# ami-iit/paper_gorbani_2025_humanoids_multi-rate-mpc-ironcub

Measured on AMD Instinct MI355X. Metric: MPC solves/sec (whole node) + p50 single-solve latency, iRonCub paper horizon, higher is better.
Workload: dtype f64

## Files before the change

### paper_gorbani_2025_humanoids_multi-rate-mpc-ironcub_amd/build.py

```python
from __future__ import annotations

import os
import shutil
import subprocess

HERE = os.path.dirname(os.path.abspath(__file__))
CSRC = os.path.join(HERE, "csrc")
LIB_PATH = os.path.join(HERE, "libvsmpc.so")
SOLVE = "vsmpc_kernels.hip"
SOURCES = [SOLVE, "vsmpc_dispatch.hip", "vsmpc_rollout.hip", "vsmpc_capi.hip", "vsmpc_jet.hip", "vsmpc_provider.hip",
           "vsmpc_runtime.hip"]
HEADERS = ["vsmpc_device.hpp", "vsmpc_launch.hpp", "vsmpc_p0.hpp", "vsmpc_smem.hpp", "vsmpc_p1_syrk.hpp", "vsmpc_p1_struct.hpp",
           "vsmpc_p3.hpp", "vsmpc_p4.hpp", "vsmpc_p5.hpp", "vsmpc_panel_asm.inc",
           "vsmpc_runtime_body.inc", "vsmpc_jet_device.hpp", "vsmpc_horizons.def", os.path.join("..", "..", "include", "vsmpc.h"),
           os.path.join("..", "..", "include", "vsmpc_jet.h")]


DEFAULT_HORIZONS = ((17, 7, 12), (34, 14, 24), (21, 9, 15))
HORIZONS_DEF = os.path.join(CSRC, "vsmpc_horizons.def")


def horizons():
    env = os.environ.get("VSMPC_HORIZONS", "").strip()
    if not env:
# ... 25 lines not shown


OBJ_DIR = os.path.join(HERE, "build")


SCHED_MAX_ILP = ["-mllvm", "-amdgpu-sched-strategy=max-ilp"]


def _units():
    units = []
    for n, ns, hc in horizons():
        sched = SCHED_MAX_ILP if n <= 24 else []
        for st in (0, 1):
            units.append((f"kernels_{n}_{ns}_{hc}_{'diag' if st else 'prod'}", SOLVE,
                          [f"-DVS_TU_HORIZON={n},{ns},{hc}", f"-DVS_TU_STAMPS={st}"] + sched))
    for src in SOURCES:
        if src != SOLVE:
            units.append((os.path.splitext(src)[0], src, []))
    return units


def _deps(src):
    return [os.path.join(CSRC, src)] + [os.path.join(CSRC, h) for h in HEADERS] + [os.path.abspath(__file__)]


def _extra_flags():
    return os.environ.get("VSMPC_HIPCC_FLAGS", "").split()


def needs_build() -> bool:
# ... 80 lines not shown
```

### paper_gorbani_2025_humanoids_multi-rate-mpc-ironcub_amd/csrc/vsmpc_capi.hip

```cpp
#include <algorithm>
#include <cmath>
#include <cstddef>
#include <cstdio>
#include <cstdlib>
#include <cstring>
#include <new>
#include <vector>

#include "vsmpc_launch.hpp"
#include "../../include/vsmpc_jet.h"

using namespace vsmpc;

struct vsmpc_handle {
    vsmpc_config cfg;
    DevCfg dev;
    int variant;
    int runtime;
    RtDims rt;
    double* d_ws;
    int sens;
    RtDims rts;
    double* d_sws;
    double* d_sdx;
    double* d_sdfm;
    int* d_sact;
    int* d_sflags;
    int form;
    KinOpts kin;
    int device;
    int max_batch;
    int n_var, n_con, n_in, n_p;
    double* d_in;
    double* d_x;
    double* d_fm;
    int* d_status;
    int* d_iters;
    double* d_lin;
    double* d_dbg;
    double* d_kin;
    double* d_kout;
    unsigned long long* d_stamps;
    hipEvent_t ev0, ev1;
// ... 57 lines not shown
}

#define HIP_TRY(expr)                                   \
    do {                                                \
        hipError_t _e = (expr);                         \
        if (_e != hipSuccess) return hip_fail(_e, #expr); \
    } while (0)

#define ON_DEVICE(dev) DeviceScope _scope(dev); HIP_TRY(_scope.err)

hipError_t solve_launch(const vsmpc_handle* h, const double* d_in, int batch, double* d_x, double* d_fm, int* d_status,
                        int* d_iters, size_t first, hipStream_t s) {
    if (h->runtime)
        return launch_solve_runtime(h->rt, h->dev, d_in, batch, h->d_ws + first * size_t(h->rt.ws_doubles), d_x, d_fm,
                                    d_status, d_iters, s);
    return launch_solve(h->variant, h->form, h->dev, d_in, batch, d_x, d_fm, d_status, d_iters, nullptr, nullptr, nullptr, s);
}

struct Stage {
    double* in; double* x; double* fm; int* st; int* it; double* kin;
};
Stage stage_view(const vsmpc_handle* h, double* base) {
    Stage v;
    v.in = base;
    v.x = v.in + size_t(ZC_MAX) * h->n_in;
    v.fm = v.x + size_t(ZC_MAX) * h->n_var;
    v.st = reinterpret_cast<int*>(v.fm + size_t(ZC_MAX) * VSMPC_FM_SIZE);
    v.it = v.st + ZC_MAX;
    v.kin = v.fm + size_t(ZC_MAX) * (VSMPC_FM_SIZE + 1);
    return v;
// ... 181 lines not shown
        if (h->pipe_done[i]) (void)hipEventDestroy(h->pipe_done[i]);
    }
    if (h->pipe_start) (void)hipEventDestroy(h->pipe_start);
    if (h->h_stage) (void)hipHostFree(h->h_stage);
    if (h->ev0) (void)hipEventDestroy(h->ev0);
    if (h->ev1) (void)hipEventDestroy(h->ev1);
    delete h;
}

int vsmpc_num_variables(const vsmpc_handle* h) { return h ? h->n_var : VSMPC_ERR_INVALID_ARG; }
int vsmpc_num_constraints(const vsmpc_handle* h) { return h ? h->n_con : VSMPC_ERR_INVALID_ARG; }
int vsmpc_input_doubles(const vsmpc_handle* h) { return h ? h->n_in : VSMPC_ERR_INVALID_ARG; }
int vsmpc_max_batch(const vsmpc_handle* h) { return h ? h->max_batch : VSMPC_ERR_INVALID_ARG; }
int vsmpc_condensed_dim(const vsmpc_handle* h) { return h ? h->n_p : VSMPC_ERR_INVALID_ARG; }
const char* vsmpc_kernel_name(const vsmpc_handle* h) {
    return h ? (h->runtime ? runtime_kernel_name() : variant_kernel_name(h->variant)) : "none";
}

int vsmpc_solve_batch_device(vsmpc_handle* h, const double* d_in, int batch, double* d_x, double* d_first_move,
                             int* d_status, int* d_iters, void* stream) {
    if (h == nullptr || d_in == nullptr || d_status == nullptr || batch < 0) return VSMPC_ERR_INVALID_ARG;
    if (batch > h->max_batch) return VSMPC_ERR_BATCH_TOO_LARGE;
    if (batch == 0) return VSMPC_OK;
    ON_DEVICE(h->device);
    HIP_TRY(solve_launch(h, d_in, batch, d_x, d_first_move, d_status, d_iters, 0, static_cast<hipStream_t>(stream)));
    return VSMPC_OK;
}

int vsmpc_solve_batch(vsmpc_handle* h, const double* in, int batch, double* x, double* first_move, int* status,
                      int* iters, void* stream) {
    if (h == nullptr || in == nullptr || status == nullptr || batch < 0) return VSMPC_ERR_INVALID_ARG;
// ... 216 lines not shown
            } else {
                lo[r1 + i * NTH + r] = h->dev.vmin;
                hi[r1 + i * NTH + r] = h->dev.vmax;
            }
        }
    return VSMPC_OK;
}

int vsmpc_debug_condensed(vsmpc_handle* h, const double* in_one, double* M, double* Lfac) {
    if (h == nullptr || in_one == nullptr) return VSMPC_ERR_INVALID_ARG;
    if (h->runtime) return VSMPC_ERR_UNSUPPORTED_CONFIG;
    ON_DEVICE(h->device);
    const size_t np2 = size_t(h->n_p) * h->n_p;
    HIP_TRY(hipMemcpy(h->d_in, in_one, h->n_in * sizeof(double), hipMemcpyHostToDevice));
    HIP_TRY(hipMemset(h->d_dbg, 0, 2 * np2 * sizeof(double)));
    HIP_TRY(launch_solve(h->variant, h->form, h->dev, h->d_in, 1, h->d_x, h->d_fm, h->d_status, h->d_iters, h->d_dbg,
                         h->d_dbg + np2, nullptr, nullptr));
    HIP_TRY(hipDeviceSynchronize());
    if (M) HIP_TRY(hipMemcpy(M, h->d_dbg, np2 * sizeof(double), hipMemcpyDeviceToHost));
    if (Lfac) HIP_TRY(hipMemcpy(Lfac, h->d_dbg + np2, np2 * sizeof(double), hipMemcpyDeviceToHost));
    return VSMPC_OK;
}

int vsmpc_kinematics_batch(vsmpc_handle* h, const double* kin, int batch, double* out, double* records) {
    if (h == nullptr || kin == nullptr || out == nullptr || batch < 0) return VSMPC_ERR_INVALID_ARG;
    if (batch > h->max_batch) return VSMPC_ERR_BATCH_TOO_LARGE;
    if (batch == 0) return VSMPC_OK;
    ON_DEVICE(h->device);
    HIP_TRY(hipMemcpy(h->d_kin, kin, size_t(batch) * VSMPC_KIN_SIZE * sizeof(double), hipMemcpyHostToDevice));
    HIP_TRY(launch_kinematics(h->d_kin, batch, h->d_kout, h->kin, nullptr));
// ... 85 lines not shown
            if (joint_selector[i] < 0 || joint_selector[i] >= VSMPC_KIN_NJ) return VSMPC_ERR_INVALID_ARG;
        for (int i = 0; i < VSMPC_N_JOINTS; ++i) h->kin.sel[i] = joint_selector[i];
    }
    h->kin.constant_lambda = constant_lambda ? 1 : 0;
    return VSMPC_OK;
}

int vsmpc_debug_phase_cycles(vsmpc_handle* h, const double* in, int batch, unsigned long long* stamps16) {
    if (h == nullptr || in == nullptr || stamps16 == nullptr || batch <= 0) return VSMPC_ERR_INVALID_ARG;
    if (h->runtime) return VSMPC_ERR_UNSUPPORTED_CONFIG;
    if (batch > h->max_batch) return VSMPC_ERR_BATCH_TOO_LARGE;
    ON_DEVICE(h->device);
    unsigned long long* d_st = h->d_stamps;
    HIP_TRY(hipMemset(d_st, 0, size_t(batch) * 16 * sizeof(unsigned long long)));
    HIP_TRY(hipMemcpy(h->d_in, in, size_t(batch) * h->n_in * sizeof(double), hipMemcpyHostToDevice));
    for (int rep = 0; rep < 3; ++rep)
        HIP_TRY(launch_solve(h->variant, h->form, h->dev, h->d_in, batch, h->d_x, h->d_fm, h->d_status, h->d_iters, nullptr,
                             nullptr, d_st, nullptr));
    HIP_TRY(hipDeviceSynchronize());
    HIP_TRY(hipMemcpy(stamps16, d_st, size_t(batch) * 16 * sizeof(unsigned long long), hipMemcpyDeviceToHost));
    return VSMPC_OK;
}

int vsmpc_timing_begin(vsmpc_handle* h, void* stream) {
    if (h == nullptr) return VSMPC_ERR_INVALID_ARG;
    HIP_TRY(hipEventRecord(h->ev0, static_cast<hipStream_t>(stream)));
    return VSMPC_OK;
}

int vsmpc_timing_end(vsmpc_handle* h, void* stream, int launches, float* ms_per_launch) {
// ... 250 lines not shown
int vsmpc_rollout_get_state(vsmpc_rollout* r, double* state) {
    if (r == nullptr || state == nullptr) return VSMPC_ERR_INVALID_ARG;
    ON_DEVICE(r->h->device);
    HIP_TRY(hipMemcpy(state, r->d_state, size_t(r->batch) * VSMPC_PLANT_STATE * sizeof(double), hipMemcpyDeviceToHost));
    return VSMPC_OK;
}

int vsmpc_rollout_get_records(vsmpc_rollout* r, double* records) {
    if (r == nullptr || records == nullptr) return VSMPC_ERR_INVALID_ARG;
    ON_DEVICE(r->h->device);
    HIP_TRY(hipMemcpy(records, r->d_rec, size_t(r->batch) * r->h->n_in * sizeof(double), hipMemcpyDeviceToHost));
    return VSMPC_OK;
}

int vsmpc_set_kernel_form(vsmpc_handle* h, int form) {
    if (h == nullptr || form < 0 || form > 2) return VSMPC_ERR_INVALID_ARG;
    if (h->runtime && form != 0) return VSMPC_ERR_UNSUPPORTED_CONFIG;
    if (form == 1 && !variant_has_structured(h->variant)) return VSMPC_ERR_UNSUPPORTED_CONFIG;
    const int prev = h->form;
    h->form = form;
    return prev;
}

void* vsmpc_alloc_host(size_t bytes) {
    void* p = nullptr;
    if (bytes == 0 || hipHostMalloc(&p, bytes, hipHostMallocDefault) != hipSuccess) { (void)hipGetLastError(); return nullptr; }
    return p;
}

void vsmpc_free_host(void* p) {
    if (p != nullptr) (void)hipHostFree(p);
}

// ... 14 lines not shown
```

### paper_gorbani_2025_humanoids_multi-rate-mpc-ironcub_amd/csrc/vsmpc_dispatch.hip

```cpp
#include <cstdlib>

#include "vsmpc_launch.hpp"
#include "vsmpc_smem.hpp"

namespace vsmpc {

__global__ __launch_bounds__(64) void kinematics_kernel(const double* __restrict__ kin, int batch,
                                                        double* __restrict__ out, KinOpts opts) {
    __shared__ __attribute__((aligned(16))) double s[VSMPC_KIN_SIZE + 1];
    __shared__ double sRa[12], sRr[12];
    const int b = blockIdx.x, lane = threadIdx.x;
    if (b >= batch) return;
    const double* rec = kin + size_t(b) * VSMPC_KIN_SIZE;
    const int head = (reinterpret_cast<size_t>(rec) & 15) ? 1 : 0;
    if (lane == 0 && head) s[0] = rec[0];
    const double2* r2 = reinterpret_cast<const double2*>(rec + head);
    const int n2 = (VSMPC_KIN_SIZE - head) / 2;
    for (int i = lane; i < n2; i += 64) {
        const double2 v = r2[i];
        s[head + 2 * i] = v.x;
        s[head + 2 * i + 1] = v.y;
    }
    if (lane == 0 && ((VSMPC_KIN_SIZE - head) & 1)) s[VSMPC_KIN_SIZE - 1] = rec[VSMPC_KIN_SIZE - 1];
    __syncthreads();
// ... 65 lines not shown
hipError_t launch_kinematics(const double* d_kin, int batch, double* d_out, const KinOpts& opts, hipStream_t stream) {
    hipLaunchKernelGGL(kinematics_kernel, dim3(batch), dim3(64), 0, stream, d_kin, batch, d_out, opts);
    return hipGetLastError();
}

int initial_kernel_form() {
    const char* v = getenv("VSMPC_FORM");
    return (v != nullptr && v[0] == 's' && v[1] == 't') ? 1 : (v != nullptr && v[0] == 's' && v[1] == 'y') ? 2 : 0;
}

struct HorizonEntry {
    int n_iter, n_iter_small, control_horizon, n_p;
    size_t lds_bytes;
    const char* name;
    bool structured;
};
#define VSMPC_STR2(x) #x
#define VSMPC_STR(x) VSMPC_STR2(x)
static const HorizonEntry kHorizons[] = {
#define X(N, NS, HC) {N, NS, HC, Dims<N, NS, HC>::NP, Dims<N, NS, HC>::STRUCT_P1 ? Smem<Dims<N, NS, HC>>::bytes_struct : Smem<Dims<N, NS, HC>>::bytes, "solve_kernel<Dims<" VSMPC_STR(N) "," VSMPC_STR(NS) "," VSMPC_STR(HC) ">>", Dims<N, NS, HC>::STRUCT_P1},
#include "vsmpc_horizons.def"
#undef X
};
constexpr int kNumHorizons = int(sizeof(kHorizons) / sizeof(kHorizons[0]));

int select_variant(int n_iter, int n_iter_small, int control_horizon) {
    for (int i = 0; i < kNumHorizons; ++i)
        if (kHorizons[i].n_iter == n_iter && kHorizons[i].n_iter_small == n_iter_small &&
            kHorizons[i].control_horizon == control_horizon)
            return i + 1;
    return VARIANT_NONE;
}

int num_variants() { return kNumHorizons; }

void variant_horizon(int variant, int* n_iter, int* n_iter_small, int* control_horizon) {
    const HorizonEntry& h = kHorizons[variant - 1];
    *n_iter = h.n_iter;
    *n_iter_small = h.n_iter_small;
    *control_horizon = h.control_horizon;
}

const char* variant_kernel_name(int variant) {
    return (variant >= 1 && variant <= kNumHorizons) ? kHorizons[variant - 1].name : "none";
}

int variant_condensed_dim(int variant) {
    return (variant >= 1 && variant <= kNumHorizons) ? kHorizons[variant - 1].n_p : 0;
}

bool variant_has_structured(int variant) {
    return variant >= 1 && variant <= kNumHorizons && kHorizons[variant - 1].structured;
}

size_t variant_lds_bytes(int variant) {
    return (variant >= 1 && variant <= kNumHorizons) ? kHorizons[variant - 1].lds_bytes : 0;
}

hipError_t launch_solve(int variant, int form, const DevCfg& cfg, const double* d_in, int batch, double* d_x, double* d_fm,
                        int* d_status, int* d_iters, double* dbgM, double* dbgL, unsigned long long* stamps,
                        hipStream_t stream) {
    int id = 0;
#define X(N, NS, HC)                                                                                                  \
// ... 24 lines not shown
```

### paper_gorbani_2025_humanoids_multi-rate-mpc-ironcub_amd/csrc/vsmpc_kernels.hip

```cpp
#include <atomic>

#include "vsmpc_launch.hpp"
#include "vsmpc_p0.hpp"
#include "vsmpc_p1_syrk.hpp"
#include "vsmpc_p1_struct.hpp"
#include "vsmpc_p3.hpp"
#include "vsmpc_p4.hpp"
#include "vsmpc_p5.hpp"

#if !defined(VS_TU_HORIZON) || !defined(VS_TU_STAMPS)
#error "one unit per horizon: -DVS_TU_HORIZON=N,NS,HC -DVS_TU_STAMPS=0|1 (build.py)"
#endif

namespace vsmpc {

template <class D, int K0 = 0, int K1 = NJC>
VS_DEV void p0_joint_reduction(double* __restrict__ sm, int lane) {
    using S = Smem<D>;
    static_assert(VSMPC_IN_LANG == VSMPC_IN_LLIN + 24, "Lambda_lin and Lambda_ang are adjacent in the record");
    const double* sIn = sm + S::oIn;
    const double* sCfg = sm + S::oCfg;
    double* sBj = sm + S::oBj;
    double* sQR = sm + S::oQR;
    const int c = lane < 6 ? lane : 6;
    double a[8];
    if constexpr (K0 == 0) {
// ... 117 lines not shown
    double* xout;
    double* fmout;
    int* status_out;
    int* iters_out;
    double* dbgM;
    double* dbgL;
    unsigned long long* stamps;
};
VS_DEV const SolveArgs* late_args() {
    const SolveArgs* ka = reinterpret_cast<const SolveArgs*>(
        (const void*)__builtin_amdgcn_kernarg_segment_ptr());
    asm volatile("" : "+s"(ka));
    return ka;
}

template <class D, bool STAMPS, int FORM = 0>
__global__ __launch_bounds__(D::BLOCK, D::WG_PER_CU) void solve_kernel(DevCfg cfg, const double* __restrict__ in, int batch,
                                                         double* xout_, double* fmout_, int* status_out_,
                                                         int* iters_out_, double* dbgM_, double* dbgL_,
                                                         unsigned long long* stamps_) {
#define VS_STAMP(i)                                                                         \
    do {                                                                                    \
        if constexpr (STAMPS) {                                                             \
            unsigned long long* st_ = late_args()->stamps;                                  \
            if (tid == 0 && st_ != nullptr) st_[size_t(blockIdx.x) * 16 + (i)] = __builtin_amdgcn_s_memtime(); \
        }                                                                                   \
    } while (0)
    unsigned long long t_acc[6] = {0, 0, 0, 0, 0, 0};
    unsigned long long t_mark = 0, stamp_t1 = 0, rt0 = 0;
    if constexpr (STAMPS) rt0 = __builtin_amdgcn_s_memrealtime();
#define VS_TIC()                                                     \
    do {                                                             \
        if constexpr (STAMPS) t_mark = __builtin_amdgcn_s_memtime(); \
    } while (0)
#define VS_TOC(i)                                                          \
    do {                                                                   \
        if constexpr (STAMPS) {                                            \
            const unsigned long long t_now = __builtin_amdgcn_s_memtime(); \
            t_acc[i] += t_now - t_mark;                                    \
            t_mark = t_now;                                                \
        }                                                                  \
    } while (0)
    using S = Smem<D>;
    constexpr bool FUSED_DISPATCH = FORM == 1;
    constexpr bool PIPE = FORM == 1;
    constexpr int QR_P0_STEPS = D::STRUCT_LONG ? 1 : 2;
    extern __shared__ __attribute__((aligned(16))) double smem[];
    double* sIn = smem + S::oIn;
    double* sA = smem + S::oA;
    double* sBj = smem + S::oBj;
    double* sBt = smem + S::oBt;
    double* sC = smem + S::oC;
    double* sVprev = smem + S::oVprev;
    double* sInvD = smem + S::oInvD;
    double* sW = smem + S::oW;
    double* sZ = smem + S::oZ;
    double* sSv = smem + S::oSv;
    double* sSvec = smem + S::oSvec;
    double* sV = smem + S::oV;
    double* sX = smem + S::oX;
// ... 32 lines not shown
        if (tid < D::NIN / 2) rec = in2[tid];
        if (tid < 4) sFlags[tid] = 0;
        if (tid < D::N) sDt[tid] = cfg.dt[tid];
        if (tid >= 64 && tid < 64 + NWROWS) sCfg[CFG_SQ + tid - 64] = cfg.sq[tid - 64];
        if (tid >= 96 && tid < 96 + NJ) sCfg[CFG_WJ + tid - 96] = cfg.wj[tid - 96];
        if (tid == 128) {
            sCfg[CFG_WREG] = cfg.w_reg; sCfg[CFG_WTHR] = cfg.w_thr; sCfg[CFG_WINIT] = cfg.w_init;
            sCfg[CFG_VMIN] = cfg.vmin; sCfg[CFG_VMAX] = cfg.vmax;
        }
        for (int i = tid; i < NX * NX + NX * NJ + NX * NTH + 28; i += D::BLOCK) sA[i] = 0.0;
        if (tid < D::NIN / 2) sIn2[tid] = rec;
    }
    __syncthreads();
    p0_linearize<D, false, false, false>(cfg.use_jet, sIn, sA, sBj, sBt, sC, sVprev, tid, D::BLOCK);
    if (wave == 3) {
        if constexpr (FORM == 1) p0_joint_reduction<D, 0, QR_P0_STEPS>(smem, lane);
        else p0_joint_reduction<D>(smem, lane);
    }

    constexpr int NJROW = D::NV + NTH + 1, ZROW = D::NV + NTH;
    double* sJetT = sXinv;
    double* sGA = sJetT + NJROW * D::N;
    static_assert(D::NV + NTH <= 64 && NJROW * D::N + 6 * D::N <= S::NXT * D::TS, "jet trajectories fit the X region");
    if (wave == 1) {
        if (lane < D::NV + NTH) {
            const bool affl = lane >= D::NV;
            const int i = affl ? lane - D::NV : (lane & 3);
            const int blk = affl ? -1 : v_block_of_internal<D>(lane);
            const double jon = sA[(12 + i) * NX + 16 + i], ja = sA[(16 + i) * NX + 12 + i], jb = sA[(16 + i) * NX + 16 + i];
            const double c12 = sC[12 + i], c16 = sC[16 + i], b12 = sBt[(12 + i) * NTH + i], b16 = sBt[(16 + i) * NTH + i];
            const double t0 = sIn[VSMPC_IN_X0 + 12 + i], td0 = sIn[VSMPC_IN_X0 + 16 + i];
            const double bT = affl ? c12 : b12, bTd = affl ? c16 : b16;
            double T = affl ? t0 : 0.0, Td = affl ? td0 : 0.0;
#pragma unroll
            for (int k = 0; k < D::N; ++k) {
                sJetT[lane * D::N + k] = T;
                const double mT = (affl || throttle_block_of_stage<D>(k) == blk) ? 1.0 : 0.0;
                const double dT = fma(jon, Td, mT * bT);
                const double dTd = fma(ja, T, fma(jb, Td, mT * bTd));
                const double dt = sDt[k];
                T = fma(dt, dT, T);
                Td = fma(dt, dTd, Td);
            }
        }
        for (int k = lane; k < D::N; k += 64) sJetT[ZROW * D::N + k] = 0.0;
        if constexpr (FORM == 1) {
            const double am = sIn[VSMPC_IN_ALPHA] * sIn[VSMPC_IN_MASS];
            const double* R = sIn + VSMPC_IN_WRB;
            const double* gr = sIn + VSMPC_IN_GRAV;
            for (int e = lane; e < 6 * D::N; e += 64) {
                const int h = e / (3 * D::N), k = (e / 3) % D::N, r = e % 3;
                double g = 0.0;
#pragma unroll
                for (int c = 0; c < NTH; ++c) g = fma(sIn[VSMPC_IN_AMOM + (3 * h + r) * NTH + c], sJetT[(D::NV + c) * D::N + k], g);
                const double ch = h == 0 ? am * (R[0 + r] * gr[0] + R[3 + r] * gr[1] + R[6 + r] * gr[2]) : 0.0;
                sGA[e] = g + ch;
            }
        }
    }
    if constexpr (FORM == 1) {
        if (wave == 2) {
            for (int e = lane; e < S::sizeZero; e += 64) smem[S::oSZero + e] = 0.0;
            for (int e = lane; e < 12 * D::NREF; e += 64) {
                const int row = e % 12;
                const double off = row < 3 ? -sIn[VSMPC_IN_PREF + row] : ((row >= 6 && row < 9) ? -sIn[VSMPC_IN_RPYINIT + row - 6] : 0.0);
                smem[S::oSRefC + e] = sIn[VSMPC_IN_XREF + e] + off;
            }
        }
    }
    if constexpr (FORM == 1 && D::STRUCT_LONG) {
        for (int e = tid; e < S::sizeAc; e += D::BLOCK) smem[S::oSAc + e] = 0.0;
    }
    __syncthreads();
    if constexpr (FORM != 1) {
        for (int e = tid; e < 6 * D::N; e += D::BLOCK) {
            const int h = e / (3 * D::N), k = (e / 3) % D::N, r = e % 3, row = (h ? 9 : 3) + r;
            double g = 0.0;
#pragma unroll
            for (int c = 0; c < NTH; ++c) g = fma(sA[row * NX + 12 + c], sJetT[(D::NV + c) * D::N + k], g);
            sGA[e] = g;
        }
        __syncthreads();
    }

    VS_STAMP(1);
    VS_REFRESH_IDS();
    if constexpr (STAMPS) stamp_t1 = __builtin_amdgcn_s_memtime();
    d4 acc[TPW];
    if constexpr (FORM == 1) {
        static_assert(D::STRUCT_P1, "structured condensing is instantiated for horizons with Dims::STRUCT_P1");
        VS_TIC();
        if (wave < 2) {
            p1s_chain<D, 0>(cfg, wave, lane, smem);
            if (wave == 0) p0_joint_reduction<D, QR_P0_STEPS, NJC>(smem, lane);
        } else {
            p1s_chain<D, 1>(cfg, wave - 2, lane, smem);
        }
        VS_TOC(0);
        __syncthreads();
        VS_TOC(1);
        if constexpr (!D::STRUCT_LONG) {
            p1s_contract<D>(smem, tid);
            __syncthreads();
        }
// ... 293 lines not shown
        for (int e = tid; e < (D::NP - 16 * PVT) * (D::NP - 16 * PVT); e += D::BLOCK) {
            const int gr = 16 * PVT + e / (D::NP - 16 * PVT), gc = 16 * PVT + e % (D::NP - 16 * PVT);
            if (gc <= gr) dbgLi[size_t(gr) * D::NP + gc] = Lb[lower_at<D>(gr, gc)];
        }
    }

    VS_STAMP(4);
    VS_REFRESH_IDS();
    if constexpr (D::WG_PER_CU == 1) pin_tiles_agpr<TPW>(acc);
    const bool hold = sIn[VSMPC_IN_HOLD] != 0.0;
    constexpr int PV = D::PVT;
    auto init_corner_rhs = [&]() {
        if (tid >= 16 * PV && tid < D::NP) sW[tid] = tid < D::NZ ? -Lb[lower_at<D>(D::NZ, tid)] : 0.0;
    };
    init_corner_rhs();
    if (tid < D::NP) sZ[tid] = (hold && tid >= D::NZ - 4 && tid < D::NZ) ? sVprev[tid - (D::NZ - 4)] : 0.0;
    __syncthreads();

    auto sweep_tile = [&](int p, bool prescribed) {
        if (wave == 0) {
            const int j = lane & 15;
            const int gj = 16 * p + j;
            const double* Tpp = Lb + tile_off<D>(p, p) + j;
            double colv[16];
#pragma unroll
            for (int k = 0; k < 16; ++k) {
                const double t = Tpp[k * 17];
                colv[k] = k >= j ? t : 0.0;
            }
            double w = sW[gj];
// ... 48 lines not shown
            const bool fix = (j >= KL) || (hold && j >= KL - 4);
            const double inv_eff = fix ? 0.0 : sInvD[gj];
            const double zadd = (fix && j < KL) ? sZ[gj] : 0.0;
            double z = 0.0;
#pragma unroll
            for (int k = KL - 1; k >= 0; --k) {
                const double zk = readlane_f64(fma(w, inv_eff, zadd), k);
                z = (j == k) ? zk : z;
                w = fma(-colv[k], zk, w);
                w6 = fma(-l76[k], zk, w6);
            }
            double z6 = 0.0;
#pragma unroll
            for (int i = 0; i < 16; ++i) z6 = fma(x6[i], readlane_f64(w6, i), z6);
            if (lane < 16) { sZ[gj] = z; sZ[16 * PV + j] = z6; }
        }
    } else if constexpr (S::DUAL3) {
        static_assert(D::NT - 1 == PV + 2, "three throttle tile rows");
        double x2[16];
        const double* L22d = Lb + tile_off_c<D>(PV + 2, PV + 2);
        const double* inv2 = sInvD + D::NU + 32;
        if (wave == 1) tile_inverse_rows<0, 8>(L22d, inv2, x2, lane);
        sweep_tile(PV + 2, false);
        auto sweep_tile_x = [&](int p, const double* Xp) {
            if (wave == 0) {
                const int j = lane & 15;
                double z0 = 0.0, z1 = 0.0;
#pragma unroll
                for (int k = 0; k < 16; k += 2) {
                    z0 = fma(Xp[k * 17 + j], sW[16 * p + k], z0);
// ... 27 lines not shown
    } else {
#pragma unroll 1
        for (int p = D::NT - 1; p >= PV; --p) sweep_tile(p, false);
    }
    if (wave == 0) {
        const bool valid = lane < D::NV;
        const double v = sZ[D::NU + (valid ? lane : 0)];
        const bool fixed = hold && lane >= D::NV - 4;
        const double tolv = 1e-12 * (1.0 + fabs(v));
        const bool viol = valid && !fixed && (v < sCfg[CFG_VMIN] - tolv || v > sCfg[CFG_VMAX] + tolv);
        const unsigned long long vm = __ballot(viol);
        if (lane == 0) { sFlags[3] = __popcll(vm); sFlags[1] = VSMPC_STATUS_SOLVED; sFlags[2] = 1; }
    }
    __syncthreads();
    const bool need_qp = sFlags[3] != 0;
    VS_STAMP(5);
    VS_REFRESH_IDS();

    if (need_qp) {
        box_qp<D>(sFlags[3], hold, wave);
        __syncthreads();
        VS_STAMP(6);
        VS_REFRESH_IDS();
        if constexpr (D::NU % 16 != 0) {
            init_corner_rhs();
            __syncthreads();
#pragma unroll 1
            for (int p = D::NT - 1; p >= PV; --p) sweep_tile(p, true);
        }
    } else {
        VS_STAMP(6);
    }
    switch (wave) {
        case 0:
            if constexpr (PIPE) p5_wave0_jets<D>(smem, lane);
// ... 214 lines not shown
    }
    if (tid == 0) {
        int st = sFlags[1];
        if (sFlags[0]) st = VSMPC_STATUS_NUMERICAL;
        status_out[inst] = st;
        if (iters_out != nullptr) iters_out[inst] = sFlags[2];
    }
    VS_P6_TOC(3);
    VS_STAMP(9);
    if constexpr (STAMPS) {
        unsigned long long* st_ = late_args()->stamps;
        if (tid == 0 && st_ != nullptr) {
#if defined(VS_DIAG_P3) && !defined(VS_DIAG_P6)
            for (int i = 0; i < 4; ++i) t_acc[i] = vs_diag_p3[i];
#endif
            t_acc[5] = __builtin_amdgcn_s_memrealtime() - rt0;
            t_acc[4] = rt0;
            for (int i = 0; i < 6; ++i) st_[size_t(blockIdx.x) * 16 + 10 + i] = t_acc[i];
        }
    }
#undef VS_STAMP
#undef VS_REFRESH_IDS
#undef VS_TIC
#undef VS_TOC
}

constexpr int MAX_DEVICES = 64;

template <class D, bool STAMPS, int FORM>
static hipError_t launch_solve_f(int dev, const DevCfg& cfg, const double* d_in, int batch, double* d_x, double* d_fm,
                                 int* d_status, int* d_iters, double* dbgM, double* dbgL,
                                 unsigned long long* stamps, hipStream_t stream) {
    static std::atomic<bool> attr_set[MAX_DEVICES];
    constexpr size_t lds = FORM == 1 ? Smem<D>::bytes_struct : Smem<D>::bytes;
    if (!attr_set[dev].load(std::memory_order_acquire)) {
        hipError_t e = hipFuncSetAttribute(reinterpret_cast<const void*>(&solve_kernel<D, STAMPS, FORM>),
                                           hipFuncAttributeMaxDynamicSharedMemorySize, int(lds));
        if (e != hipSuccess) return e;
        attr_set[dev].store(true, std::memory_order_release);
    }
    hipLaunchKernelGGL((solve_kernel<D, STAMPS, FORM>), dim3(batch), dim3(D::BLOCK), lds, stream,
                       cfg, d_in, batch, d_x, d_fm, d_status, d_iters, dbgM, dbgL, stamps);
    return hipGetLastError();
}

template <int N, int NS, int HC, bool STAMPS>
hipError_t launch_solve_dims(int form, const DevCfg& cfg, const double* d_in, int batch, double* d_x, double* d_fm,
                             int* d_status, int* d_iters, double* dbgM, double* dbgL, unsigned long long* stamps,
                             hipStream_t stream) {
    using D = Dims<N, NS, HC>;
    int dev = 0;
    hipError_t e = hipGetDevice(&dev);
    if (e != hipSuccess) return e;
    if (dev < 0 || dev >= MAX_DEVICES) return hipErrorInvalidDevice;
    if constexpr (D::STRUCT_P1) {
        if (form != 2) {
            return launch_solve_f<D, STAMPS, 1>(dev, cfg, d_in, batch, d_x, d_fm, d_status, d_iters, dbgM, dbgL, stamps,
                                                stream);
        }
    }
    return launch_solve_f<D, STAMPS, 0>(dev, cfg, d_in, batch, d_x, d_fm, d_status, d_iters, dbgM, dbgL, stamps,
                                            stream);
}

template <int N, int NS, int HC>
hipError_t launch_linearize_dims(const DevCfg& cfg, const double* d_in, int batch, double* A, double* Bj, double* Bt,
                                 double* c, hipStream_t stream) {
    hipLaunchKernelGGL((linearize_kernel<Dims<N, NS, HC>>), dim3(batch), dim3(256), 0, stream, cfg, d_in, A, Bj, Bt, c);
    return hipGetLastError();
}

#define VS_INSTANTIATE_SOLVE(N, NS, HC, ST)                                                                              \
    template hipError_t launch_solve_dims<N, NS, HC, ST>(int, const DevCfg&, const double*, int, double*, double*, int*, \
                                                         int*, double*, double*, unsigned long long*, hipStream_t);
#define VS_INSTANTIATE_LIN(N, NS, HC)                                                                                   \
    template hipError_t launch_linearize_dims<N, NS, HC>(const DevCfg&, const double*, int, double*, double*, double*, \
                                                         double*, hipStream_t);
#define VS_TU_APPLY(M, ...) M(__VA_ARGS__)
#if VS_TU_STAMPS
VS_TU_APPLY(VS_INSTANTIATE_SOLVE, VS_TU_HORIZON, true)
#else
VS_TU_APPLY(VS_INSTANTIATE_SOLVE, VS_TU_HORIZON, false)
VS_TU_APPLY(VS_INSTANTIATE_LIN, VS_TU_HORIZON)
#endif

}
```

### paper_gorbani_2025_humanoids_multi-rate-mpc-ironcub_amd/csrc/vsmpc_launch.hpp

```cpp
#pragma once
#include <hip/hip_runtime.h>

#include "vsmpc_device.hpp"

struct vsmpc_jet;

namespace vsmpc {

struct DeviceScope {
    int caller = -1, target = -1;
    hipError_t err = hipSuccess;
    explicit DeviceScope(int device) : target(device) {
        err = hipGetDevice(&caller);
        if (err == hipSuccess && caller != target) err = hipSetDevice(target);
    }
    ~DeviceScope() { if (caller >= 0 && caller != target) (void)hipSetDevice(caller); }
    DeviceScope(const DeviceScope&) = delete;
    DeviceScope& operator=(const DeviceScope&) = delete;
};

enum Variant { VARIANT_NONE = 0 };

int select_variant(int n_iter, int n_iter_small, int control_horizon);
int num_variants();
void variant_horizon(int variant, int* n_iter, int* n_iter_small, int* control_horizon);
const char* variant_kernel_name(int variant);
int variant_condensed_dim(int variant);
size_t variant_lds_bytes(int variant);

int initial_kernel_form();
bool variant_has_structured(int variant);

hipError_t launch_solve(int variant, int form, const DevCfg& cfg, const double* d_in, int batch, double* d_x, double* d_fm,
                        int* d_status, int* d_iters, double* dbgM, double* dbgL, unsigned long long* stamps,
                        hipStream_t stream);
hipError_t launch_linearize(int variant, const DevCfg& cfg, const double* d_in, int batch, double* A, double* Bj,
                            double* Bt, double* c, hipStream_t stream);
template <int N, int NS, int HC, bool STAMPS>
hipError_t launch_solve_dims(int form, const DevCfg& cfg, const double* d_in, int batch, double* d_x, double* d_fm,
                             int* d_status, int* d_iters, double* dbgM, double* dbgL, unsigned long long* stamps,
                             hipStream_t stream);
template <int N, int NS, int HC>
hipError_t launch_linearize_dims(const DevCfg& cfg, const double* d_in, int batch, double* A, double* Bj, double* Bt,
                                 double* c, hipStream_t stream);

struct RtDims {
    int n, ns, hc;
    int nvb, nu, nv;
    int nz, np;
    int nin, nxs, nvar;
    int ntri;
    int ws_doubles;
    int lds_doubles;
};
constexpr size_t RT_MAX_LDS = 160 * 1024;
RtDims runtime_dims(int n_iter, int n_iter_small, int control_horizon, bool sensitivity = false);
// ... 58 lines not shown
```

### paper_gorbani_2025_humanoids_multi-rate-mpc-ironcub_amd/csrc/vsmpc_p4.hpp

```cpp
#pragma once
#include "vsmpc_smem.hpp"

namespace vsmpc {

template <int K, int NVS>
VS_DEV double small_spd_solve(const double* __restrict__ sP, unsigned long long mask, double rhs, int lane, int& bad) {
    int idx[K];
#pragma unroll
    for (int q = 0; q < K; ++q) {
        idx[q] = __ffsll((long long)mask) - 1;
        mask &= mask - 1;
    }
    double A[K][K], d[K];
#pragma unroll
    for (int q = 0; q < K; ++q) {
        d[q] = readlane_f64(rhs, idx[q]);
#pragma unroll
        for (int c = 0; c <= q; ++c) A[q][c] = sP[idx[c] * NVS + idx[q]];
    }
    double ip[K];
#pragma unroll
    for (int j = 0; j < K; ++j) {
        bad |= !(A[j][j] > 0.0);
        ip[j] = fast_rcp(A[j][j]);
// ... 236 lines not shown
        const int ninf = __popcll(imask);
        if (ninf == 0) { status = VSMPC_STATUS_SOLVED; break; }
        bool pick = inf;
        if (ninf < best) { best = ninf; patience = AS_PATIENCE; }
        else if (patience > 0) { --patience; }
        else { pick = inf && (lane == 63 - __clzll(imask)); }
        if (pick) state = vlo ? -1 : (vhi ? 1 : 0);
    }
    if (valid) {
        v = fixed ? lo : (state < 0 ? lo : (state > 0 ? hi : v));
        sZ[D::NU + lane] = v;
    }
    if (lane == 0) { sFlags[1] = status; sFlags[2] = iters; }
}

template <class D>
VS_DEV void box_qp(int n_violated, bool hold, int wave) {
    using S = Smem<D>;
    extern __shared__ __attribute__((aligned(16))) double smem[];
    double* sVprev = smem + S::oVprev;
    double* sInvD = smem + S::oInvD;
    double* sZ = smem + S::oZ;
    double* sSv = smem + S::oSv;
    double* sSvec = smem + S::oSvec;
    double* sCfg = smem + S::oCfg;
    int* sFlags = reinterpret_cast<int*>(smem + S::oFlags);
    double* Lb = smem + S::oM;
    double* sXinv = smem + S::oXinv;
    double* sQP = smem + S::oQP;
    const int lane = fresh_lane(), tid = (wave << 6) | lane;
    constexpr bool DUALQP = S::DUALQP;
    constexpr int PV = D::PVT;
    constexpr int DUAL_MAX_ACTIVE = 16;
    constexpr bool DUAL3 = S::DUAL3;
    constexpr int DUAL3_MAX = 24;
    const bool few = n_violated <= (DUAL3 ? DUAL3_MAX : DUAL_MAX_ACTIVE);
    (void)sQP; (void)sXinv; (void)sInvD;
      if (few && DUALQP) {
       if constexpr (DUALQP) {
        {
            constexpr int NVS = D::NV + 1, NR2 = D::NV - 16;
            double* sXr = sQP + D::NV * NVS;
            double* sT = sQP;
            const double* X6 = sXinv + PV * D::TS;
            const double* L76 = Lb + tile_off<D>(PV + 1, PV);
            const double* L77 = Lb + tile_off<D>(PV + 1, PV + 1);
            constexpr int XT0 = 17 * NR2 <= 192 ? 16 * NR2 : 224;
            static_assert(XT0 + NR2 <= D::BLOCK && D::NV <= 32, "threads of the X77 columns");
            if (tid < 16 * NR2) {
                const int a2 = tid >> 4, j = tid & 15;
                double t0 = 0.0, t1 = 0.0;
#pragma unroll
                for (int k = 0; k < 16; k += 2) {
                    t0 = fma(L76[a2 * 17 + k], X6[k * 17 + j], t0);
                    t1 = fma(L76[a2 * 17 + k + 1], X6[(k + 1) * 17 + j], t1);
// ... 17 lines not shown
            __syncthreads();
            if (wave == 3) {
                double gm = 0.0;
#pragma unroll
                for (int c = 0; c < D::NV; ++c) gm = fmax(gm, fabs(sSvec[c]));
                if (lane == 0) sSvec[0] = gm;
            }
            if (tid < 16 * NR2) {
                const int a2 = tid >> 4, j = tid & 15;
                double t = 0.0;
#pragma unroll
                for (int b2 = 0; b2 < NR2; ++b2) t = fma(sXr[a2 * NVS + 16 + b2], sT[b2 * 16 + j], t);
                sXr[a2 * NVS + j] = -t;
            }
            __syncthreads();
        }
        static_assert(D::NU % 16 == 0 && D::NV > 16 && D::NV <= 32, "throttle block: tile aligned, two tile rows");
        const XTiles<D> xa{sXinv + PV * D::TS, sQP + D::NV * (D::NV + 1)};
        const bool all_cols = n_violated > 4;
        if (all_cols) {
            const int n = hold ? D::NV - 4 : D::NV;
            for (int e = tid; e < D::NV * D::NV; e += D::BLOCK) {
                const int b = e / D::NV, r = e - b * D::NV;
                sSv[b * (D::NV + 1) + r] = xa.pcol(b, r, n);
            }
            __syncthreads();
        }
        if (wave == 0)
            dual_active_set<D>(xa, hold, lane, sSv, sQP, sSvec, sVprev, sCfg, sZ, sFlags, all_cols ? ((1ull << D::NV) - 1ull) : 0ull);
       }
// ... 230 lines not shown
```

### paper_gorbani_2025_humanoids_multi-rate-mpc-ironcub_amd/solver.py

```python
from __future__ import annotations

import ctypes

import numpy as np

from . import _lib
from . import layout as L
from .jet_model import JetModel


def _ptr(a):
    return None if a is None else a.ctypes.data_as(ctypes.c_void_p)


KERNEL_FORM_AUTO, KERNEL_FORM_STRUCTURED, KERNEL_FORM_SYRK = 0, 1, 2


class BatchedVSMPC:

    def __init__(self, cfg: L.MPCConfig | None = None, device: int = 0, max_batch: int = 256, runtime: str = "never",
                 sensitivity: bool = False):
        if runtime not in L.RUNTIME_MODES:
            raise ValueError(f"runtime must be one of {sorted(L.RUNTIME_MODES)}, not {runtime!r}")
        self.cfg = cfg or L.paper_config()
        self.lib = _lib.load()
        self._ccfg = self.cfg.to_c()
        self._h = ctypes.c_void_p()
        if runtime == "never" and not sensitivity:
            _lib.check(self.lib.vsmpc_create(ctypes.byref(self._ccfg), device, max_batch, ctypes.byref(self._h)),
                       "vsmpc_create")
# ... 270 lines not shown
```

Baseline: 7.508 million.

## Add lone-block kernel variant that overlaps box-QP setup with triangular sweep

Adds a FORM_LONE instantiation of the structured solve kernel, chosen automatically when the batch fits within the CU count. In that case the box-QP Schur setup (the T and X77 products and the Schur right-hand side) runs on idle waves during the corner triangular solve, so box_qp can skip its own setup phase and a barrier. The aim is lower single-solve latency at small batches. It also adds a compile unit per horizon, a CU-count query, diagnostic timing hooks, and a form 3 that forces the two-per-CU kernel.

```diff
diff --git a/paper_gorbani_2025_humanoids_multi-rate-mpc-ironcub_amd/build.py b/paper_gorbani_2025_humanoids_multi-rate-mpc-ironcub_amd/build.py
--- a/paper_gorbani_2025_humanoids_multi-rate-mpc-ironcub_amd/build.py
+++ b/paper_gorbani_2025_humanoids_multi-rate-mpc-ironcub_amd/build.py
@@ -63,6 +63,8 @@
         for st in (0, 1):
             units.append((f"kernels_{n}_{ns}_{hc}_{'diag' if st else 'prod'}", SOLVE,
                           [f"-DVS_TU_HORIZON={n},{ns},{hc}", f"-DVS_TU_STAMPS={st}"] + sched))
+            units.append((f"kernels_{n}_{ns}_{hc}_lone_{'diag' if st else 'prod'}", SOLVE,
+                          [f"-DVS_TU_HORIZON={n},{ns},{hc}", f"-DVS_TU_STAMPS={st}", "-DVS_TU_LONE=1"] + sched))
     for src in SOURCES:
         if src != SOLVE:
             units.append((os.path.splitext(src)[0], src, []))
diff --git a/paper_gorbani_2025_humanoids_multi-rate-mpc-ironcub_amd/csrc/vsmpc_capi.hip b/paper_gorbani_2025_humanoids_multi-rate-mpc-ironcub_amd/csrc/vsmpc_capi.hip
--- a/paper_gorbani_2025_humanoids_multi-rate-mpc-ironcub_amd/csrc/vsmpc_capi.hip
+++ b/paper_gorbani_2025_humanoids_multi-rate-mpc-ironcub_amd/csrc/vsmpc_capi.hip
@@ -27,6 +27,7 @@
     int* d_sact;
     int* d_sflags;
     int form;
+    mutable int last_batch;
     KinOpts kin;
     int device;
     int max_batch;
@@ -114,6 +115,7 @@
     if (h->runtime)
         return launch_solve_runtime(h->rt, h->dev, d_in, batch, h->d_ws + first * size_t(h->rt.ws_doubles), d_x, d_fm,
                                     d_status, d_iters, s);
+    h->last_batch = batch;
     return launch_solve(h->variant, h->form, h->dev, d_in, batch, d_x, d_fm, d_status, d_iters, nullptr, nullptr, nullptr, s);
 }
 
@@ -325,7 +327,9 @@
 int vsmpc_max_batch(const vsmpc_handle* h) { return h ? h->max_batch : VSMPC_ERR_INVALID_ARG; }
 int vsmpc_condensed_dim(const vsmpc_handle* h) { return h ? h->n_p : VSMPC_ERR_INVALID_ARG; }
 const char* vsmpc_kernel_name(const vsmpc_handle* h) {
-    return h ? (h->runtime ? runtime_kernel_name() : variant_kernel_name(h->variant)) : "none";
+    if (h == nullptr) return "none";
+    if (h->runtime) return runtime_kernel_name();
+    return solve_kernel_name(h->variant, h->form, h->last_batch > 0 ? h->last_batch : h->max_batch, h->device);
 }
 
 int vsmpc_solve_batch_device(vsmpc_handle* h, const double* d_in, int batch, double* d_x, double* d_first_move,
@@ -572,6 +576,7 @@
     const size_t np2 = size_t(h->n_p) * h->n_p;
     HIP_TRY(hipMemcpy(h->d_in, in_one, h->n_in * sizeof(double), hipMemcpyHostToDevice));
     HIP_TRY(hipMemset(h->d_dbg, 0, 2 * np2 * sizeof(double)));
+    h->last_batch = 1;
     HIP_TRY(launch_solve(h->variant, h->form, h->dev, h->d_in, 1, h->d_x, h->d_fm, h->d_status, h->d_iters, h->d_dbg,
                          h->d_dbg + np2, nullptr, nullptr));
     HIP_TRY(hipDeviceSynchronize());
@@ -687,6 +692,7 @@
     unsigned long long* d_st = h->d_stamps;
     HIP_TRY(hipMemset(d_st, 0, size_t(batch) * 16 * sizeof(unsigned long long)));
     HIP_TRY(hipMemcpy(h->d_in, in, size_t(batch) * h->n_in * sizeof(double), hipMemcpyHostToDevice));
+    h->last_batch = batch;
     for (int rep = 0; rep < 3; ++rep)
         HIP_TRY(launch_solve(h->variant, h->form, h->dev, h->d_in, batch, h->d_x, h->d_fm, h->d_status, h->d_iters, nullptr,
                              nullptr, d_st, nullptr));
@@ -967,9 +973,9 @@
 }
 
 int vsmpc_set_kernel_form(vsmpc_handle* h, int form) {
-    if (h == nullptr || form < 0 || form > 2) return VSMPC_ERR_INVALID_ARG;
+    if (h == nullptr || form < 0 || form > 3) return VSMPC_ERR_INVALID_ARG;
     if (h->runtime && form != 0) return VSMPC_ERR_UNSUPPORTED_CONFIG;
-    if (form == 1 && !variant_has_structured(h->variant)) return VSMPC_ERR_UNSUPPORTED_CONFIG;
+    if ((form == 1 || form == 3) && !variant_has_structured(h->variant)) return VSMPC_ERR_UNSUPPORTED_CONFIG;
     const int prev = h->form;
     h->form = form;
     return prev;
diff --git a/paper_gorbani_2025_humanoids_multi-rate-mpc-ironcub_amd/csrc/vsmpc_dispatch.hip b/paper_gorbani_2025_humanoids_multi-rate-mpc-ironcub_amd/csrc/vsmpc_dispatch.hip
--- a/paper_gorbani_2025_humanoids_multi-rate-mpc-ironcub_amd/csrc/vsmpc_dispatch.hip
+++ b/paper_gorbani_2025_humanoids_multi-rate-mpc-ironcub_amd/csrc/vsmpc_dispatch.hip
@@ -1,3 +1,4 @@
+#include <atomic>
 #include <cstdlib>
 
 #include "vsmpc_launch.hpp"
@@ -103,11 +104,14 @@
     size_t lds_bytes;
     const char* name;
     bool structured;
+    const char* lone_name;
 };
+template <class D>
+constexpr bool kHorizonHasLone = D::STRUCT_P1 && !D::STRUCT_LONG && D::WG_PER_CU == 2;
 #define VSMPC_STR2(x) #x
 #define VSMPC_STR(x) VSMPC_STR2(x)
 static const HorizonEntry kHorizons[] = {
-#define X(N, NS, HC) {N, NS, HC, Dims<N, NS, HC>::NP, Dims<N, NS, HC>::STRUCT_P1 ? Smem<Dims<N, NS, HC>>::bytes_struct : Smem<Dims<N, NS, HC>>::bytes, "solve_kernel<Dims<" VSMPC_STR(N) "," VSMPC_STR(NS) "," VSMPC_STR(HC) ">>", Dims<N, NS, HC>::STRUCT_P1},
+#define X(N, NS, HC) {N, NS, HC, Dims<N, NS, HC>::NP, Dims<N, NS, HC>::STRUCT_P1 ? Smem<Dims<N, NS, HC>>::bytes_struct : Smem<Dims<N, NS, HC>>::bytes, "solve_kernel<Dims<" VSMPC_STR(N) "," VSMPC_STR(NS) "," VSMPC_STR(HC) ">>", Dims<N, NS, HC>::STRUCT_P1, kHorizonHasLone<Dims<N, NS, HC>> ? "solve_kernel<Dims<" VSMPC_STR(N) "," VSMPC_STR(NS) "," VSMPC_STR(HC) ">, lone>" : nullptr},
 #include "vsmpc_horizons.def"
 #undef X
 };
@@ -136,6 +140,31 @@
 
 int variant_condensed_dim(int variant) {
     return (variant >= 1 && variant <= kNumHorizons) ? kHorizons[variant - 1].n_p : 0;
+}
+
+bool variant_has_lone(int variant) {
+    return variant >= 1 && variant <= kNumHorizons && kHorizons[variant - 1].lone_name != nullptr;
+}
+
+int device_cu_count(int device) {
+    constexpr int MAX_DEVICES = 64;
+    static std::atomic<int> cus[MAX_DEVICES];
+    if (device < 0 || device >= MAX_DEVICES) return 0;
+    int n = cus[device].load(std::memory_order_acquire);
+    if (n == 0) {
+        if (hipDeviceGetAttribute(&n, hipDeviceAttributeMultiprocessorCount, device) != hipSuccess || n < 0) {
+            (void)hipGetLastError();
+            return 0;
+        }
+        cus[device].store(n, std::memory_order_release);
+    }
+    return n;
+}
+
+const char* solve_kernel_name(int variant, int form, int batch, int device) {
+    if (variant_has_lone(variant) && form != 2 && form != 3 && batch <= device_cu_count(device))
+        return kHorizons[variant - 1].lone_name;
+    return variant_kernel_name(variant);
 }
 
 bool variant_has_structured(int variant) {
diff --git a/paper_gorbani_2025_humanoids_multi-rate-mpc-ironcub_amd/csrc/vsmpc_kernels.hip b/paper_gorbani_2025_humanoids_multi-rate-mpc-ironcub_amd/csrc/vsmpc_kernels.hip
--- a/paper_gorbani_2025_humanoids_multi-rate-mpc-ironcub_amd/csrc/vsmpc_kernels.hip
+++ b/paper_gorbani_2025_humanoids_multi-rate-mpc-ironcub_amd/csrc/vsmpc_kernels.hip
@@ -9,7 +9,10 @@
 #include "vsmpc_p5.hpp"
 
 #if !defined(VS_TU_HORIZON) || !defined(VS_TU_STAMPS)
-#error "one unit per horizon: -DVS_TU_HORIZON=N,NS,HC -DVS_TU_STAMPS=0|1 (build.py)"
+#error "one unit per horizon: -DVS_TU_HORIZON=N,NS,HC -DVS_TU_STAMPS=0|1 [-DVS_TU_LONE=1] (build.py)"
+#endif
+#ifndef VS_TU_LONE
+#define VS_TU_LONE 0
 #endif
 
 namespace vsmpc {
@@ -157,6 +160,9 @@
     return ka;
 }
 
+constexpr int FORM_LONE = 3;
+template <class D>
+constexpr bool kHasLone = D::STRUCT_P1 && !D::STRUCT_LONG && D::WG_PER_CU == 2;
 template <class D, bool STAMPS, int FORM = 0>
 __global__ __launch_bounds__(D::BLOCK, D::WG_PER_CU) void solve_kernel(DevCfg cfg, const double* __restrict__ in, int batch,
                                                          double* xout_, double* fmout_, int* status_out_,
@@ -185,8 +191,10 @@
         }                                                                  \
     } while (0)
     using S = Smem<D>;
-    constexpr bool FUSED_DISPATCH = FORM == 1;
-    constexpr bool PIPE = FORM == 1;
+    constexpr bool LONE = FORM == FORM_LONE;
+    constexpr bool STRUCT = FORM == 1 || LONE;
+    constexpr bool FUSED_DISPATCH = STRUCT;
+    constexpr bool PIPE = STRUCT;
     constexpr int QR_P0_STEPS = D::STRUCT_LONG ? 1 : 2;
     extern __shared__ __attribute__((aligned(16))) double smem[];
     double* sIn = smem + S::oIn;
@@ -249,7 +257,7 @@
     __syncthreads();
     p0_linearize<D, false, false, false>(cfg.use_jet, sIn, sA, sBj, sBt, sC, sVprev, tid, D::BLOCK);
     if (wave == 3) {
-        if constexpr (FORM == 1) p0_joint_reduction<D, 0, QR_P0_STEPS>(smem, lane);
+        if constexpr (STRUCT) p0_joint_reduction<D, 0, QR_P0_STEPS>(smem, lane);
         else p0_joint_reduction<D>(smem, lane);
     }
 
@@ -279,7 +287,7 @@
             }
         }
         for (int k = lane; k < D::N; k += 64) sJetT[ZROW * D::N + k] = 0.0;
-        if constexpr (FORM == 1) {
+        if constexpr (STRUCT) {
             const double am = sIn[VSMPC_IN_ALPHA] * sIn[VSMPC_IN_MASS];
             const double* R = sIn + VSMPC_IN_WRB;
             const double* gr = sIn + VSMPC_IN_GRAV;
@@ -293,7 +301,7 @@
             }
         }
     }
-    if constexpr (FORM == 1) {
+    if constexpr (STRUCT) {
         if (wave == 2) {
             for (int e = lane; e < S::sizeZero; e += 64) smem[S::oSZero + e] = 0.0;
             for (int e = lane; e < 12 * D::NREF; e += 64) {
@@ -303,11 +311,11 @@
             }
         }
     }
-    if constexpr (FORM == 1 && D::STRUCT_LONG) {
+    if constexpr (STRUCT && D::STRUCT_LONG) {
         for (int e = tid; e < S::sizeAc; e += D::BLOCK) smem[S::oSAc + e] = 0.0;
     }
     __syncthreads();
-    if constexpr (FORM != 1) {
+    if constexpr (!STRUCT) {
         for (int e = tid; e < 6 * D::N; e += D::BLOCK) {
             const int h = e / (3 * D::N), k = (e / 3) % D::N, r = e % 3, row = (h ? 9 : 3) + r;
             double g = 0.0;
@@ -322,7 +330,7 @@
     VS_REFRESH_IDS();
     if constexpr (STAMPS) stamp_t1 = __builtin_amdgcn_s_memtime();
     d4 acc[TPW];
-    if constexpr (FORM == 1) {
+    if constexpr (STRUCT) {
         static_assert(D::STRUCT_P1, "structured condensing is instantiated for horizons with Dims::STRUCT_P1");
         VS_TIC();
         if (wave < 2) {
@@ -646,6 +654,10 @@
         if (tid >= 16 * PV && tid < D::NP) sW[tid] = tid < D::NZ ? -Lb[lower_at<D>(D::NZ, tid)] : 0.0;
     };
     init_corner_rhs();
+#ifdef VS_DIAG_QP
+    if (tid < 4) vs_diag_qp[tid] = 0;
+    const unsigned long long qp_sweep0 = __builtin_amdgcn_s_memtime();
+#endif
     if (tid < D::NP) sZ[tid] = (hold && tid >= D::NZ - 4 && tid < D::NZ) ? sVprev[tid - (D::NZ - 4)] : 0.0;
     __syncthreads();
 
@@ -724,6 +736,8 @@
 #pragma unroll
             for (int i = 0; i < 16; ++i) z6 = fma(x6[i], readlane_f64(w6, i), z6);
             if (lane < 16) { sZ[gj] = z; sZ[16 * PV + j] = z6; }
+        } else if constexpr (LONE) {
+            box_qp_setup_lone<D>(wave);
         }
     } else if constexpr (S::DUAL3) {
         static_assert(D::NT - 1 == PV + 2, "three throttle tile rows");
@@ -781,11 +795,14 @@
     }
     __syncthreads();
     const bool need_qp = sFlags[3] != 0;
+#ifdef VS_DIAG_QP
+    if (tid == 0) vs_diag_qp[2] = __builtin_amdgcn_s_memtime() - qp_sweep0;
+#endif
     VS_STAMP(5);
     VS_REFRESH_IDS();
 
     if (need_qp) {
-        box_qp<D>(sFlags[3], hold, wave);
+        box_qp<D, LONE && DUALQP>(sFlags[3], hold, wave);
         __syncthreads();
         VS_STAMP(6);
         VS_REFRESH_IDS();
@@ -1030,6 +1047,9 @@
 #if defined(VS_DIAG_P3) && !defined(VS_DIAG_P6)
             for (int i = 0; i < 4; ++i) t_acc[i] = vs_diag_p3[i];
 #endif
+#if defined(VS_DIAG_QP) && !defined(VS_DIAG_P3) && !defined(VS_DIAG_P6)
+            for (int i = 0; i < 3; ++i) t_acc[i] = vs_diag_qp[i];
+#endif
             t_acc[5] = __builtin_amdgcn_s_memrealtime() - rt0;
             t_acc[4] = rt0;
             for (int i = 0; i < 6; ++i) st_[size_t(blockIdx.x) * 16 + 10 + i] = t_acc[i];
@@ -1048,7 +1068,7 @@
                                  int* d_status, int* d_iters, double* dbgM, double* dbgL,
                                  unsigned long long* stamps, hipStream_t stream) {
     static std::atomic<bool> attr_set[MAX_DEVICES];
-    constexpr size_t lds = FORM == 1 ? Smem<D>::bytes_struct : Smem<D>::bytes;
+    constexpr size_t lds = (FORM == 1 || FORM == FORM_LONE) ? Smem<D>::bytes_struct : Smem<D>::bytes;
     if (!attr_set[dev].load(std::memory_order_acquire)) {
         hipError_t e = hipFuncSetAttribute(reinterpret_cast<const void*>(&solve_kernel<D, STAMPS, FORM>),
                                            hipFuncAttributeMaxDynamicSharedMemorySize, int(lds));
@@ -1060,6 +1080,28 @@
     return hipGetLastError();
 }
 
+#if VS_TU_LONE
+template <int N, int NS, int HC, bool STAMPS>
+hipError_t launch_solve_lone_dims(const DevCfg& cfg, const double* d_in, int batch, double* d_x, double* d_fm, int* d_status,
+                                  int* d_iters, double* dbgM, double* dbgL, unsigned long long* stamps, hipStream_t stream) {
+    using D = Dims<N, NS, HC>;
+    if constexpr (kHasLone<D>) {
+        int dev = 0;
+        hipError_t e = hipGetDevice(&dev);
+        if (e != hipSuccess) return e;
+        if (dev < 0 || dev >= MAX_DEVICES) return hipErrorInvalidDevice;
+        return launch_solve_f<D, STAMPS, FORM_LONE>(dev, cfg, d_in, batch, d_x, d_fm, d_status, d_iters, dbgM, dbgL, stamps,
+                                                    stream);
+    } else {
+        return hipErrorInvalidValue;
+    }
+}
+#define VS_INSTANTIATE_LONE(N, NS, HC, ST)                                                                                 \
+    template hipError_t launch_solve_lone_dims<N, NS, HC, ST>(const DevCfg&, const double*, int, double*, double*, int*, \
+                                                              int*, double*, double*, unsigned long long*, hipStream_t);
+#define VS_TU_APPLY(M, ...) M(__VA_ARGS__)
+VS_TU_APPLY(VS_INSTANTIATE_LONE, VS_TU_HORIZON, bool(VS_TU_STAMPS))
+#else
 template <int N, int NS, int HC, bool STAMPS>
 hipError_t launch_solve_dims(int form, const DevCfg& cfg, const double* d_in, int batch, double* d_x, double* d_fm,
                              int* d_status, int* d_iters, double* dbgM, double* dbgL, unsigned long long* stamps,
@@ -1071,6 +1113,11 @@
     if (dev < 0 || dev >= MAX_DEVICES) return hipErrorInvalidDevice;
     if constexpr (D::STRUCT_P1) {
         if (form != 2) {
+            if constexpr (kHasLone<D>) {
+                if (form != 3 && batch <= device_cu_count(dev))
+                    return launch_solve_lone_dims<N, NS, HC, STAMPS>(cfg, d_in, batch, d_x, d_fm, d_status, d_iters, dbgM, dbgL,
+                                                                     stamps, stream);
+            }
             return launch_solve_f<D, STAMPS, 1>(dev, cfg, d_in, batch, d_x, d_fm, d_status, d_iters, dbgM, dbgL, stamps,
                                                 stream);
         }
@@ -1099,5 +1146,6 @@
 VS_TU_APPLY(VS_INSTANTIATE_SOLVE, VS_TU_HORIZON, false)
 VS_TU_APPLY(VS_INSTANTIATE_LIN, VS_TU_HORIZON)
 #endif
+#endif
 
 }
diff --git a/paper_gorbani_2025_humanoids_multi-rate-mpc-ironcub_amd/csrc/vsmpc_launch.hpp b/paper_gorbani_2025_humanoids_multi-rate-mpc-ironcub_amd/csrc/vsmpc_launch.hpp
--- a/paper_gorbani_2025_humanoids_multi-rate-mpc-ironcub_amd/csrc/vsmpc_launch.hpp
+++ b/paper_gorbani_2025_humanoids_multi-rate-mpc-ironcub_amd/csrc/vsmpc_launch.hpp
@@ -31,6 +31,10 @@
 int initial_kernel_form();
 bool variant_has_structured(int variant);
 
+bool variant_has_lone(int variant);
+int device_cu_count(int device);
+const char* solve_kernel_name(int variant, int form, int batch, int device);
+
 hipError_t launch_solve(int variant, int form, const DevCfg& cfg, const double* d_in, int batch, double* d_x, double* d_fm,
                         int* d_status, int* d_iters, double* dbgM, double* dbgL, unsigned long long* stamps,
                         hipStream_t stream);
@@ -40,6 +44,9 @@
 hipError_t launch_solve_dims(int form, const DevCfg& cfg, const double* d_in, int batch, double* d_x, double* d_fm,
                              int* d_status, int* d_iters, double* dbgM, double* dbgL, unsigned long long* stamps,
                              hipStream_t stream);
+template <int N, int NS, int HC, bool STAMPS>
+hipError_t launch_solve_lone_dims(const DevCfg& cfg, const double* d_in, int batch, double* d_x, double* d_fm, int* d_status,
+                                  int* d_iters, double* dbgM, double* dbgL, unsigned long long* stamps, hipStream_t stream);
 template <int N, int NS, int HC>
 hipError_t launch_linearize_dims(const DevCfg& cfg, const double* d_in, int batch, double* A, double* Bj, double* Bt,
                                  double* c, hipStream_t stream);
diff --git a/paper_gorbani_2025_humanoids_multi-rate-mpc-ironcub_amd/csrc/vsmpc_p4.hpp b/paper_gorbani_2025_humanoids_multi-rate-mpc-ironcub_amd/csrc/vsmpc_p4.hpp
--- a/paper_gorbani_2025_humanoids_multi-rate-mpc-ironcub_amd/csrc/vsmpc_p4.hpp
+++ b/paper_gorbani_2025_humanoids_multi-rate-mpc-ironcub_amd/csrc/vsmpc_p4.hpp
@@ -274,7 +274,78 @@
     if (lane == 0) { sFlags[1] = status; sFlags[2] = iters; }
 }
 
+#ifdef VS_DIAG_QP
+__shared__ unsigned long long vs_diag_qp[4];
+#endif
 template <class D>
+VS_DEV void box_qp_setup_lone(int wave) {
+    using S = Smem<D>;
+    static_assert(S::DUALQP, "the lone variant is instantiated for horizons with the two-tile-row dual box QP");
+    extern __shared__ __attribute__((aligned(16))) double smem[];
+    constexpr int PV = D::PVT, NVS = D::NV + 1, NR2 = D::NV - 16;
+    static_assert(8 * NR2 <= 64 && NR2 * 16 + NR2 * NR2 <= D::NV * NVS, "one lane per entry of half of T; scratch inside K");
+    const double* sInvD = smem + S::oInvD;
+    const double* Lb = smem + S::oM;
+    double* sQP = smem + S::oQP;
+    double* sXr = sQP + D::NV * NVS;
+    double* sT = sQP;
+    const double* X6 = smem + S::oXinv + PV * D::TS;
+    const double* L76 = Lb + tile_off<D>(PV + 1, PV);
+    const double* L77 = Lb + tile_off<D>(PV + 1, PV + 1);
+    const int lane = fresh_lane();
+#ifdef VS_DIAG_QP
+    const unsigned long long q0_ = __builtin_amdgcn_s_memtime();
+#define VS_QP_SETUP_END() do { const unsigned long long d_ = __builtin_amdgcn_s_memtime() - q0_; \
+                               if (lane == 0) atomicMax(&vs_diag_qp[1], d_); } while (0)
+#else
+#define VS_QP_SETUP_END() do { } while (0)
+#endif
+    if (wave == 3) {
+        schur_rhs<D>(Lb, smem + S::oSvec, lane);
+        double* sSvec = smem + S::oSvec;
+        double gm = 0.0;
+#pragma unroll
+        for (int c = 0; c < D::NV; ++c) gm = fmax(gm, fabs(sSvec[c]));
+        if (lane == 0) sSvec[0] = gm;
+        VS_QP_SETUP_END();
+        return;
+    }
+    double* x77 = wave == 1 ? sXr + 16 : sT + NR2 * 16;
+    const int xs = wave == 1 ? NVS : NR2;
+    const int a2 = lane >> 3, j = (lane & 7) + (wave == 1 ? 0 : 8);
+    if (lane < 8 * NR2) {
+        double t0 = 0.0, t1 = 0.0;
+#pragma unroll
+        for (int k = 0; k < 16; k += 2) {
+            t0 = fma(L76[a2 * 17 + k], X6[k * 17 + j], t0);
+            t1 = fma(L76[a2 * 17 + k + 1], X6[(k + 1) * 17 + j], t1);
+        }
+        sT[a2 * 16 + j] = t0 + t1;
+    }
+    if (lane < NR2) {
+        const int c = lane;
+        double x[NR2];
+#pragma unroll
+        for (int i = 0; i < NR2; ++i) {
+            double sum = 0.0;
+#pragma unroll
+            for (int k = 0; k < i; ++k) sum = fma(L77[i * 17 + k], (k >= c) ? x[k] : 0.0, sum);
+            const double di = sInvD[D::NU + 16 + i];
+            x[i] = (i == c) ? di : ((i > c) ? -di * sum : 0.0);
+            x77[i * xs + c] = x[i];
+        }
+    }
+    if (lane < 8 * NR2) {
+        double t = 0.0;
+#pragma unroll
+        for (int b2 = 0; b2 < NR2; ++b2) t = fma(x77[a2 * xs + b2], sT[b2 * 16 + j], t);
+        sXr[a2 * NVS + j] = -t;
+    }
+    VS_QP_SETUP_END();
+#undef VS_QP_SETUP_END
+}
+
+template <class D, bool PRESET = false>
 VS_DEV void box_qp(int n_violated, bool hold, int wave) {
     using S = Smem<D>;
     extern __shared__ __attribute__((aligned(16))) double smem[];
@@ -298,7 +369,10 @@
     (void)sQP; (void)sXinv; (void)sInvD;
       if (few && DUALQP) {
        if constexpr (DUALQP) {
-        {
+        if constexpr (!PRESET) {
+#ifdef VS_DIAG_QP
+            const unsigned long long q0_ = __builtin_amdgcn_s_memtime();
+#endif
             constexpr int NVS = D::NV + 1, NR2 = D::NV - 16;
             double* sXr = sQP + D::NV * NVS;
             double* sT = sQP;
@@ -346,6 +420,9 @@
                 sXr[a2 * NVS + j] = -t;
             }
             __syncthreads();
+#ifdef VS_DIAG_QP
+            if (tid == 0) vs_diag_qp[0] = __builtin_amdgcn_s_memtime() - q0_;
+#endif
         }
         static_assert(D::NU % 16 == 0 && D::NV > 16 && D::NV <= 32, "throttle block: tile aligned, two tile rows");
         const XTiles<D> xa{sXinv + PV * D::TS, sQP + D::NV * (D::NV + 1)};
diff --git a/paper_gorbani_2025_humanoids_multi-rate-mpc-ironcub_amd/solver.py b/paper_gorbani_2025_humanoids_multi-rate-mpc-ironcub_amd/solver.py
--- a/paper_gorbani_2025_humanoids_multi-rate-mpc-ironcub_amd/solver.py
+++ b/paper_gorbani_2025_humanoids_multi-rate-mpc-ironcub_amd/solver.py
@@ -14,6 +14,7 @@
 
 
 KERNEL_FORM_AUTO, KERNEL_FORM_STRUCTURED, KERNEL_FORM_SYRK = 0, 1, 2
+KERNEL_FORM_STRUCTURED_TWO_PER_CU = 3
 
 
 class BatchedVSMPC:
```

Measured after the change: 7.545 million, median of 6. No clear change (+0.5%).
